# xulinfei1996/koordinator

Measured on AMD Instinct MI355X. Metric: pods scheduled/sec + node-evals/sec (% HBM roofline) at 5k and 100k nodes, higher is better.
Workload: dtype int64; 1 GPU; C2: 10000 pods x 5000 nodes, NodeResourcesFit(LeastAllocated cpu/mem/batch-cpu/batch-mem) + LoadAwareScheduling(defaults) + ElasticQuota(32 leaf quotas); nodes=5000, percentage_of_nodes_to_score=100, parallelism=single-gpu, batch_pods=64, candidates=32

## Files before the change

koordinator_amd/csrc/koordgpu.hip:

```cpp
#include <hip/hip_runtime.h>

#include <algorithm>
#include <chrono>
#include <cmath>
#include <condition_variable>
#include <cstdio>
#include <cstdlib>
#include <cstring>
#include <mutex>
#include <string>
#include <vector>

#include <rccl/rccl.h>

#include "ks_pass.h"
#include "ks_mono.h"
#include "ks_fq.h"
#include "ks_debug.h"
#include "ks_topo.h"
#include "ks_preempt.h"

using namespace ks;

static int64_t env_i64(const char* name, int64_t dflt, int64_t lo, int64_t hi) {
// ... 921 lines not shown
  void* numa_blob = nullptr;
  DevNuma nv{};
  DevNuma* dnv = nullptr;
  char* numa_ckpt = nullptr;
  int64_t numa_policy_nodes = 0;
  bool cpu_bind_labels = false;
  bool cpu_bind_required = false;
  bool val_bind_required = false;
  bool staged_bind_required = false;
  bool cpusets_clobbered = false;
  std::vector<int32_t> h_dev_assumed, h_dev_assumed_ckpt;
  std::vector<int8_t> h_numa_k;
  std::vector<uint16_t> h_dev_ids;
  std::vector<uint8_t> h_pol;
  std::vector<uint8_t> h_dev_held;
  bool dev_held_any = false;
  int64_t* rsv_dald_ckpt = nullptr;
  std::vector<int8_t> h_cpu_nn;
  std::vector<CpuTopo> h_topos;
  std::vector<int8_t> h_topo_dense;
  std::vector<int32_t> h_rsv_node;
  void* dscratch = nullptr;
  size_t dscratch_bytes = 0;
  uint32_t* cpuset_split = nullptr;
  hipStream_t sstream = nullptr;
  hipStream_t cstream = nullptr;
  int32_t* pipe = nullptr;
  unsigned long long* pipe_top = nullptr;
  hipEvent_t pev_sel[kPipeEvents] = {};
  hipEvent_t pev_com[kPipeEvents] = {};
  int64_t pipe_k = 0;
  int32_t pipe_mode = -1;
  bool commit_fq = true;
  void* npod_blob = nullptr;
  DevNodePods npt{};
  int32_t npod_slots = 0;
  PreemptCand* pre_cand = nullptr;
  int32_t* pre_vrank = nullptr;
  uint8_t* pre_status = nullptr;
  PreemptOut* pre_out = nullptr;
  int32_t* pre_victims = nullptr;
  int32_t topo_nkeys = 0, topo_ndom = 1, topo_nprops = 0;
  std::vector<int32_t*> topo_dom_v;
  std::vector<int32_t*> topo_count_v;
  int32_t* topo_dom = nullptr;
  int32_t* topo_count = nullptr;
  long long* topo_zsum = nullptr;
  uint32_t *topo_zpres = nullptr, *topo_zsize = nullptr;
  void* topo_blob = nullptr;
  double* topo_lw = nullptr;
  int32_t topo_nlw = 0;
  TopoScratch* topo_scr = nullptr;
  long long *topo_sraw = nullptr, *topo_iraw = nullptr;
  int32_t topo_k = 1;
  uint32_t* topo_cchunk = nullptr;
  uint2* topo_ct = nullptr;
  int32_t* topo_ccount = nullptr;
  uint64_t *topo_cbound = nullptr, *topo_ctop = nullptr, *topo_csecond = nullptr;
  ks_stats stats{};
  std::vector<hipEvent_t> ev_pool;
};

#define KS_FAIL(ctx, code, ...)                                        \
  do {                                                                 \
    char buf_[512];                                                    \
    snprintf(buf_, sizeof(buf_), __VA_ARGS__);                         \
// ... 185 lines not shown
      g_create_error = "ks_create: TaintToleration / NodeAffinity plugin weight out of range";
      return KS_EINVAL;
    }
  }
  if (cfg->reservation.enable) {
    const int64_t fitla = 100 * ((cfg->fit.enable_score ? cfg->fit.plugin_weight : 0) +
                                 (cfg->loadaware.enable_score ? cfg->loadaware.plugin_weight : 0) +
                                 (cfg->numa.enable ? cfg->numa.plugin_weight : 0) +
                                 (cfg->deviceshare.enable ? cfg->deviceshare.plugin_weight : 0) +
                                 (cfg->balanced.enable ? cfg->balanced.plugin_weight : 0) +
                                 (cfg->taint.enable_score ? cfg->taint.plugin_weight : 0) +
                                 (cfg->affinity.enable_score ? cfg->affinity.plugin_weight : 0));
    if (cfg->reservation.plugin_weight <= fitla || cfg->reservation.plugin_weight > ((int64_t)1 << 40) ||
        (fitla + 1) * (kRsvOrderBase + 1) >= (1 << 26)) {
      g_create_error = "ks_create: Reservation plugin weight must exceed 100 x (Fit + LoadAware weights) (ks_rsv.h ranking)";
      return KS_EUNSUPPORTED;
    }
  }
  int ndev = 0;
  if (hipGetDeviceCount(&ndev) != hipSuccess || ndev == 0) {
    g_create_error = "ks_create: no HIP device available";
    return KS_EHIP;
  }
  if (cfg->device < 0 || cfg->device >= ndev) {
    g_create_error = "ks_create: device ordinal out of range";
    return KS_EINVAL;
  }
  ks_ctx* ctx = new ks_ctx();
  ctx->cfg = *cfg;
  ctx->device = cfg->device;
  ctx->batch = cfg->batch_pods > 0 ? std::min(cfg->batch_pods, kMaxBatch) : 64;
  ctx->k = cfg->candidates > 0 ? std::min(cfg->candidates, kMaxCand) : 32;
  ctx->commit_fq = env_i64("KS_COMMIT_FQ", 1, 0, 1) != 0;
  if (hipSetDevice(ctx->device) != hipSuccess || hipStreamCreateWithFlags(&ctx->stream, hipStreamNonBlocking) != hipSuccess) {
    g_create_error = "ks_create: cannot create HIP stream";
    delete ctx;
    return KS_EHIP;
  }
  void* p = nullptr;
  size_t cand_bytes = (size_t)2 * kMaxBatch * kMaxCand;
  if (dev_alloc(ctx, &p, cand_bytes * 4) != KS_OK) goto fail;
  ctx->cand_chunk = (uint32_t*)p;
  if (dev_alloc(ctx, &p, cand_bytes * 8) != KS_OK) goto fail;
  ctx->cand_t = (uint2*)p;
  if (dev_alloc(ctx, &p, 2 * kMaxBatch * 8) != KS_OK) goto fail;
  ctx->cand_bound = (uint64_t*)p;
  if (dev_alloc(ctx, &p, 2 * kMaxBatch * 8) != KS_OK) goto fail;
  ctx->cand_top = (uint64_t*)p;
  if (dev_alloc(ctx, &p, 2 * kMaxBatch * 8) != KS_OK) goto fail;
  ctx->cand_second = (uint64_t*)p;
  if (dev_alloc(ctx, &p, (size_t)kMaxBatch * kPreRsvM * sizeof(PreRsv)) != KS_OK) goto fail;
  ctx->pre_rsv = (PreRsv*)p;
  if (dev_alloc(ctx, &p, 2 * kMaxBatch * 4) != KS_OK) goto fail;
  ctx->cand_total = (int32_t*)p;
  if (dev_alloc(ctx, &p, 2 * kMaxBatch * 4) != KS_OK) goto fail;
  ctx->cand_count = (int32_t*)p;
  if (dev_alloc(ctx, &p, 64) != KS_OK) goto fail;
  ctx->cursor = (int32_t*)p;
  if (dev_alloc(ctx, &p, 256) != KS_OK) goto fail;
  ctx->counters = (unsigned long long*)p;
  if (dev_alloc(ctx, &p, kNormRows * kMaxBatch * 8) != KS_OK) goto fail;
  ctx->dev_M = (unsigned long long*)p;
  if (hipMemsetAsync(ctx->cand_count, list_fill(), 2 * kMaxBatch * 4, ctx->stream) != hipSuccess ||
      hipMemsetAsync(ctx->cand_chunk, list_fill(), cand_bytes * 4, ctx->stream) != hipSuccess ||
      hipMemsetAsync(ctx->cand_t, list_fill(), cand_bytes * 8, ctx->stream) != hipSuccess ||
      hipStreamSynchronize(ctx->stream) != hipSuccess) {
// ... 2095 lines not shown
  ca.numa_bytes = (int32_t)numa_cache_bytes(ctx);
  ca.nv = ctx->dnv;
  ca.pipe_base = nullptr;
  ca.carry = nullptr;
  ca.pipe_follow = nullptr;
  ca.pipe_after = nullptr;
  ca.top_reset = nullptr;
  ca.pre_rsv = nullptr;
  ca.topo = ctx->cfg.topology.enable && st.topo ? 1 : 0;
  ca.topo_const = (int32_t)(100 * ctx->cfg.topology.spread_weight);
  ca.topo_rec = st.topo;
  ca.topo_props = st.topo_props;
  ca.topo_count = ctx->topo_count;
  ca.topo_npad = ctx->npad;
  ca.topo_best = ctx->topo_scr ? &ctx->topo_scr->best_total : nullptr;
  *smem = commit_layout(ctx->k, ctx->nchunks, *qcache, (size_t)ca.rsv_bytes, (size_t)ca.dev_bytes, (size_t)ca.numa_bytes,
                        ctx->q.q, kernel_feat(ctx) == 0, commit_hint_variant(ctx)).total;
  return ca;
}

static bool mono_commit(const ks_ctx* ctx, bool qcache, size_t* smem) {
  static const int64_t mode = env_i64("KS_COMMIT_GENERAL", 0, 0, 2);
  if (mode == 1 || kernel_feat(ctx) != 0 || !ctx->kc.monotone || ctx->kc.fit_most) return false;
  if (mode == 0 && ctx->kc.quota_enable) return false;
  *smem = mono_layout(ctx->k, ctx->nchunks, qcache, ctx->q.q).total;
  return *smem <= 160 * 1024;
}

static bool fq_commit(const ks_ctx* ctx, bool qcache, bool patch) {
  return ctx->commit_fq && qcache && !patch && kernel_feat(ctx) == 0 && ctx->kc.monotone && !ctx->kc.fit_most &&
         ctx->kc.quota_enable;
}

static FqLaunch fq_launcher(int nsc) { return nsc == 0 ? fq_launch_n0() : (nsc == 2 ? fq_launch_n2() : fq_launch_n4()); }

static bool pre_reserve(const ks_ctx* ctx) {
  static const int64_t env_pre = env_i64("KS_PRE_RSV", 1, 0, 1);
  return env_pre != 0 && ctx->kc.numa_pol;
}

static int commit_attr_set(ks_ctx* ctx) {
  bool qcache = false;
  const int32_t rcap = commit_rcap(ctx, &qcache);
  const size_t smem = commit_layout(ctx->k, ctx->nchunks, qcache, rsv_cache_bytes(ctx, rcap), dev_cache_bytes(ctx),
                                    numa_cache_bytes(ctx), ctx->q.q, kernel_feat(ctx) == 0, commit_hint_variant(ctx)).total;
  if (smem > 160 * 1024)
    KS_FAIL(ctx, KS_EUNSUPPORTED, "too many nodes for the commit kernel's LDS (%lld nodes, %zu B)", (long long)ctx->n, smem);
  hipError_t e = pass_launcher(kernel_feat(ctx), ctx->nsc).commit_attr(qcache, smem);
  if (e != hipSuccess) KS_FAIL(ctx, KS_EHIP, "hipFuncSetAttribute(commit LDS %zu): %s", smem, hipGetErrorString(e));
  if (fq_commit(ctx, qcache, false)) {
    e = fq_launcher(ctx->nsc).commit_attr(smem);
    if (e != hipSuccess) KS_FAIL(ctx, KS_EHIP, "hipFuncSetAttribute(fq commit LDS %zu): %s", smem, hipGetErrorString(e));
  }
  size_t msmem = 0;
  if (mono_commit(ctx, qcache, &msmem)) {
    e = pass_launcher(0, ctx->nsc).commit_mono_attr(qcache, msmem);
    if (e != hipSuccess) KS_FAIL(ctx, KS_EHIP, "hipFuncSetAttribute(mono commit LDS %zu): %s", msmem, hipGetErrorString(e));
  }
  return KS_OK;
}

static int ensure_cpuset_bufs(ks_ctx* ctx, int32_t np) {
  if (!ctx->cfg.numa.enable || ctx->cpuset_cap >= np) return KS_OK;
  void* p = ctx->cpuset_list;
  dev_free(p);
  ctx->cpuset_list = nullptr;
  const int32_t cap = std::max<int32_t>(np, 64);
  const size_t o_n = (size_t)cap * 8, o_out = o_n + 16, o_split = o_out + (size_t)cap * sizeof(CpuSet),
               o_alloc = align16(o_split + (size_t)cap * 4), bytes = o_alloc + (size_t)cap * 2 * kNumaDev * 8;
  if (dev_alloc(ctx, &p, bytes) != KS_OK) return KS_ENOMEM;
  ctx->cpuset_list = (int2*)p;
  ctx->cpuset_n = (int32_t*)((char*)p + o_n);
  ctx->cpuset_out = (CpuSet*)((char*)p + o_out);
  ctx->cpuset_split = (uint32_t*)((char*)p + o_split);
  ctx->numa_alloc = (int64_t*)((char*)p + o_alloc);
  ctx->cpuset_cap = cap;
  return KS_OK;
}

constexpr int kPipeWords = 4 + 1 + kMaxBatch;

static bool pipelined(const ks_ctx* ctx) {
  static const int64_t env_pipe = env_i64("KS_PIPE", 1, 0, 2);
  static const int64_t env_min = env_i64("KS_PIPE_MIN_NODES", 32768, 0, (int64_t)1 << 40);
  const int64_t mode = ctx->pipe_mode >= 0 ? ctx->pipe_mode : env_pipe;
// ... 468 lines not shown
  if (patch)
    if (int rc = fix(); rc != KS_OK) return rc;
  hipStream_t cs = pipe ? ctx->cstream : ctx->stream;
  if (patch) {
  } else if (pipe) {
    HIPCHK(ctx, hipEventRecord(ctx->pev_sel[k % kPipeEvents], ss));
    HIPCHK(ctx, hipStreamWaitEvent(cs, ctx->pev_sel[k % kPipeEvents], 0));
  }
  bool qcache = false;
  size_t smem = 0;
  CommitArgs ca = commit_args(ctx, ctx->st, ctx->np, ctx->batch, &qcache, &smem);
  if (pipe) {
    ca.pipe_base = base;
    ca.carry = carry;
  }
  ca.cand_chunk = cset.chunk;
  ca.cand_t = cset.t;
  ca.cand_bound = cset.bound;
  ca.cand_top = cset.top;
  ca.cand_second = cset.second;
  ca.cand_count = cset.count;
  if (patch) {
    ca.pipe_follow = ctx->pipe + ((k + 1) & 1);
    ca.pipe_after = base;
    ca.cand_top = (const uint64_t*)(ctx->pipe_top + (size_t)(k & 1) * kMaxBatch);
    ca.top_reset = ctx->pipe_top + (size_t)(k & 1) * kMaxBatch;
  }
  size_t msmem = 0;
  const bool mono = mono_commit(ctx, qcache, &msmem);
  if (!mono && !pipe && pl.reserve_pre && pre_reserve(ctx)) ca.pre_rsv = ctx->pre_rsv;
  rec(2, cs);
  if (ca.pre_rsv) HIPCHK(ctx, pl.reserve_pre(ctx->batch, cs, ca));
  if (mono) HIPCHK(ctx, pl.commit_mono(qcache, msmem, cs, ca));
  else if (fq_commit(ctx, qcache, patch)) HIPCHK(ctx, fq_launcher(ctx->nsc).commit(smem, cs, ca));
  else HIPCHK(ctx, pl.commit(qcache, smem, cs, ca));
  rec(2, cs);
  if (pipe) HIPCHK(ctx, hipEventRecord(ctx->pev_com[k % kPipeEvents], cs));
  ctx->pipe_k = k + 1;
  return cores_pass_refresh(ctx);
}

static int schedule_staged_impl(ks_ctx* ctx) {
  if (!ctx->node_blob) KS_FAIL(ctx, KS_ESTATE, "schedule before ks_load_nodes");
  HIPCHK(ctx, hipSetDevice(ctx->device));
  bind_mode(ctx, ctx->staged_bind_required);
  ctx->cpusets_clobbered = false;
  ctx->stats = ks_stats{};
  const int32_t np = ctx->np;
  if (np == 0) return KS_OK;
  {
    if (int rc = commit_attr_set(ctx); rc != KS_OK) return rc;
    hipError_t e = hipSuccess;
    const size_t sel_smem = select_smem(ctx->nchunks);
    if (sel_smem > 160 * 1024) KS_FAIL(ctx, KS_EUNSUPPORTED, "too many nodes for the select kernel's LDS (%lld nodes)", (long long)ctx->n);
    e = hipFuncSetAttribute((const void*)select_kernel, hipFuncAttributeMaxDynamicSharedMemorySize, (int)sel_smem);
    if (e != hipSuccess) KS_FAIL(ctx, KS_EHIP, "hipFuncSetAttribute(select LDS %zu): %s", sel_smem, hipGetErrorString(e));
    if (ctx->kc.dev && !ctx->kc.rsv && !ctx->kc.stat && ctx->dcache_words < (int64_t)kMaxBatch * ctx->npad) {
      void* q = ctx->dcache;
      dev_free(q);
      ctx->dcache = nullptr;
      ctx->dcache_words = 0;
      if (dev_alloc(ctx, &q, (size_t)kMaxBatch * ctx->npad * 8) != KS_OK) return KS_ENOMEM;
      ctx->dcache = (unsigned long long*)q;
      ctx->dcache_words = (int64_t)kMaxBatch * ctx->npad;
    }
    const size_t gb = (size_t)ctx->nranks * ctx->vshards * cand_slot_layout(ctx->k).bytes;
    if (ctx->nranks * ctx->vshards > 1 && ctx->gather_bytes < gb) {
// ... 111 lines not shown
  if (cs != ctx->stream) {
    HIPCHK(ctx, hipEventRecord(ctx->pev_com[0], cs));
    HIPCHK(ctx, hipStreamWaitEvent(ctx->stream, ctx->pev_com[0], 0));
  }
  if (ctx->cpu_loaded && ctx->n > 0) {
    hipLaunchKernelGGL(cpuset_kernel, dim3((unsigned)((ctx->n + 255) / 256)), dim3(256), 0, ctx->stream, ctx->cpu,
                       (const int2*)ctx->cpuset_list, (const int32_t*)ctx->cpuset_n, (const uint32_t*)ctx->cpuset_split,
                       (const PodRec*)ctx->st.recs, ctx->cpuset_out, (const uint32_t*)ctx->d.numa_flags,
                       ctx->d.cpu_cores, (int32_t)(ctx->cfg.numa.numa_scoring_strategy == KS_MOST_ALLOCATED),
                       numa_words(ctx), ctx->nv.npad, ctx->n);
    HIPCHK(ctx, hipGetLastError());
  }
  HIPCHK(ctx, hipEventRecord(t1, ctx->stream));
  unsigned long long cnt[16] = {0};
  HIPCHK(ctx, hipMemcpyAsync(cnt, ctx->counters, sizeof(cnt), hipMemcpyDeviceToHost, ctx->stream));
  HIPCHK(ctx, hipStreamSynchronize(ctx->stream));
  float ms = 0;
  (void)hipEventElapsedTime(&ms, t0, t1);
  ctx->stats.total_ms = ms;
  ctx->stats.passes = (int64_t)cnt[0];
  ctx->stats.cut_passes = (int64_t)cnt[1];
  ctx->stats.rescans = (int64_t)cnt[2];
  ctx->stats.slot_misses = (int64_t)cnt[3];
  ctx->stats.bubble_passes = (int64_t)cnt[4];
  ctx->stats.pre_reserves = (int64_t)cnt[5];
  ctx->stats.pipelined = pipe ? (pipe->patch ? 2 : 1) : 0;
  {
    bool qc = false;
    const int32_t rcap = commit_rcap(ctx, &qc);
    const CommitLayout L = commit_layout(ctx->k, ctx->nchunks, qc, rsv_cache_bytes(ctx, rcap), dev_cache_bytes(ctx),
                                         numa_cache_bytes(ctx), ctx->q.q, kernel_feat(ctx) == 0, commit_hint_variant(ctx));
    ctx->stats.commit_lds_bytes = (int64_t)L.total;
    ctx->stats.commit_helpers = L.hint ? 1 : 0;
  }
  for (int i = 0; i < 8; ++i) ctx->stats.diag[i] = (int64_t)cnt[8 + i];
  for (size_t i = 0; i + 1 < evs.size(); i += 2) {
    float e = 0;
    (void)hipEventElapsedTime(&e, ctx->ev_pool[evs[i].second], ctx->ev_pool[evs[i + 1].second]);
    if (evs[i].first == 0) {
      ctx->stats.sweep_ms += e;
      ctx->stats.sweep_launches += 1;
    } else if (evs[i].first == 1) {
      ctx->stats.select_ms += e;
    } else if (evs[i].first == 3) {
      ctx->stats.fixup_ms += e;
    } else {
      ctx->stats.commit_ms += e;
    }
  }
  int64_t b_node = 8 * 15 + 4 * 3 + (int64_t)ctx->nsc * 16 + (ctx->kc.rsv ? 8 : 0) + (ctx->kc.numa ? 16 : 0) +
                   (ctx->kc.dev ? 4 + (kDevTW + kDevQW) * 8 : 0);
  const int64_t groups = (ctx->batch + ppw - 1) / ppw;
  ctx->stats.sweep_bytes = local_chunks * 64 * b_node * groups + (int64_t)ctx->batch * sizeof(PodRec) + local_chunks * 64 * 4;
  return KS_OK;
}

int ks_schedule_staged(ks_ctx* ctx) {
  if (!ctx) return KS_EINVAL;
  return schedule_staged_impl(ctx);
}

int ks_fetch_results(ks_ctx* ctx, ks_result* out, int32_t p) {
  if (!ctx || !out || p < 0 || p > ctx->np) return ctx ? (ctx->err = "ks_fetch_results: bad args", KS_EINVAL) : KS_EINVAL;
  if (p == 0) return KS_OK;
  HIPCHK(ctx, hipMemcpyAsync(out, ctx->st.results, (size_t)p * sizeof(ks_result), hipMemcpyDeviceToHost, ctx->stream));
  HIPCHK(ctx, hipStreamSynchronize(ctx->stream));
// ... 920 lines not shown
```

koordinator_amd/csrc/ks_fq.h:

```cpp
#pragma once

#include "ks_pass.h"

namespace ks {

struct __attribute__((aligned(16))) FqPod {
  uint32_t qmeta;
  uint32_t flags;
  uint32_t qword;
  int32_t second;
  uint64_t bound, top;
};
static_assert(sizeof(FqPod) == 32, "FqPod layout");
static_assert(kMaxBatch == 64 && kMaxCand <= 64 && kQuotaLdsRows < 0xFFFF && KS_QUOTA_DIMS <= 8, "FqPod packing");

template <int NSC>
__device__ __forceinline__ uint64_t fq_rescan(const DevNodes* dnp, const Cfg& cfg, const PodRec& pod, int64_t chunk,
                                              uint64_t touched_mask, int64_t n) {
  const int lane = threadIdx.x & 63;
  const int64_t node = chunk * 64 + lane;
  asm volatile("" : "+s"(dnp));
  const DevNodes d = *dnp;
  NodeReg<NSC> r;
  load_node<NSC>(cfg, d, node, node < n, r);
  const EvalOut o = eval_pod_node<NSC, false>(cfg, pod, r);
  const bool skip = o.reasons || ((touched_mask >> lane) & 1ull);
  return wave_max_u64(skip ? 0ull : gkey(o.total, node));
}

template <int NSC>
__global__ __launch_bounds__(commit_threads(0)) void commit_fq_kernel(CommitArgs a) {
  constexpr int NT = commit_threads(0);
  extern __shared__ __attribute__((aligned(16))) unsigned char smem_raw[];
  const int32_t K = a.k;
  const CommitLayout lay = commit_layout(K, a.nchunks, true, (size_t)a.rsv_bytes, (size_t)a.dev_bytes, (size_t)a.numa_bytes,
                                         a.q.q, true, false);
  SlotRow* rows = reinterpret_cast<SlotRow*>(smem_raw + lay.rows);
  PodRec* spods = reinterpret_cast<PodRec*>(smem_raw + lay.pods);
  ks_result* sres = reinterpret_cast<ks_result*>(smem_raw + lay.res);
  int64_t* raw = reinterpret_cast<int64_t*>(smem_raw + lay.raw);
  int64_t* rawtop = reinterpret_cast<int64_t*>(smem_raw + lay.rawtop);
  int64_t* rawrun = reinterpret_cast<int64_t*>(smem_raw + lay.rawrun);
  int64_t* pqreq = reinterpret_cast<int64_t*>(smem_raw + lay.pqreq);
  uint2* cand_t = reinterpret_cast<uint2*>(smem_raw + lay.cand_t);
  uint32_t* cand_chunk = reinterpret_cast<uint32_t*>(smem_raw + lay.cand_chunk);
  FqPod* precs = reinterpret_cast<FqPod*>(smem_raw + lay.snuma);
  QuotaRowsLds qview = quota_lds(smem_raw + lay.quota, a.q.q);
  QuotaRowsLds* qlds = &qview;
  unsigned long long* touched = reinterpret_cast<unsigned long long*>(smem_raw + lay.touched);
  int2* hdesc = reinterpret_cast<int2*>(smem_raw + lay.help);
  int32_t* hpend = reinterpret_cast<int32_t*>(smem_raw + lay.help + (size_t)kMaxBatch * 8);
  int32_t* hdone = hpend + 1;
  unsigned long long* hready = reinterpret_cast<unsigned long long*>(smem_raw + lay.help + (size_t)kMaxBatch * 8 + 16);
  const int tid = threadIdx.x;
  const int lane = tid & 63;
  const int32_t cursor0 = __builtin_amdgcn_readfirstlane(*a.cursor);
  if (cursor0 >= a.total_pods) {
    if (threadIdx.x == 0) pipe_next(a, cursor0);
    return;
  }
  if (pipe_bubble(a, cursor0)) return;
  const int32_t np = topo_pass_pods(a, cursor0, min(a.batch, a.total_pods - cursor0));
  if (np == 0) return;
#ifdef KS_COMMIT_STAMPS
  uint64_t ph[8] = {0, 0, 0, 0, 0, 0, 0, 0};
  uint64_t tlast = __builtin_amdgcn_s_memtime();
#define KS_FSTAMP(i)                                   \
  do {                                                 \
    const uint64_t t_ = __builtin_amdgcn_s_memtime(); \
    ph[i] += t_ - tlast;                               \
    tlast = t_;                                        \
  } while (0)
#else
#define KS_FSTAMP(i) \
  do {               \
  } while (0)
#endif

  lds_copy<NT>(cand_chunk, a.cand_chunk, np * K, tid);
  lds_copy<NT>(cand_t, a.cand_t, np * K, tid);
  for (int32_t i = tid; i < np * KS_QUOTA_DIMS; i += NT) {
    const int32_t p = i / KS_QUOTA_DIMS, dd = i - p * KS_QUOTA_DIMS;
    pqreq[i] = a.pq.req[dd][cursor0 + p];
  }
  {
// ... 14 lines not shown
    qlds->limit[i] = a.q.limit[i];
    qlds->used[i] = a.q.used[i];
    qlds->min[i] = a.q.min[i];
    qlds->npused[i] = a.q.npused[i];
  }
  if (tid < 64 && lane < np) {
    const int32_t cnt = a.cand_count[lane];
    const uint64_t second = a.cand_second[lane];
    const uint32_t pmask = a.pq.mask[cursor0 + lane];
    const int32_t quota = a.pods[cursor0 + lane].quota;
    FqPod r;
    r.bound = a.cand_bound[lane];
    r.top = a.cand_top[lane];
    r.flags = a.pods[cursor0 + lane].flags;
    r.qmeta = 0xFFFFu;
    if (quota >= 0) {
      const int32_t pp = a.q.parent[quota];
      r.qmeta = (uint32_t)(pp < 0 ? 0xFFFF : pp) | ((a.q.limit_mask[quota] & 0xFFu) << 16) |
                ((a.q.min_mask[quota] & 0xFFu) << 24);
    }
    r.qword = (uint32_t)(quota < 0 ? 0xFFFF : quota) | ((pmask & 0xFFu) << 16) | ((uint32_t)max(0, min(cnt, 64)) << 24);
    r.second = (int32_t)gkey_node(second);
    precs[lane] = r;
  }
  const void* my_col = nullptr;
  int32_t my_w = 8;
  if (tid < RF_N) {
    my_col = a.rowcols[lane].p;
    my_w = a.rowcols[lane].width;
  }
  if (tid == 0) {
    *hpend = 0;
    *hdone = 0;
    *hready = 0ull;
  }
  __syncthreads();
  if (tid >= 128) return;
  KS_FSTAMP(0);
  Cfg cfg{};
  {
    auto pin = [](int32_t v) {
      asm volatile("" : "+s"(v));
      return v;
    };
    cfg.fit_filter = pin(a.c.fit_filter);
    cfg.fit_score = pin(a.c.fit_score);
    cfg.fw_cpu = pin(a.c.fw_cpu);
    cfg.fw_mem = pin(a.c.fw_mem);
    cfg.fw_eph = pin(a.c.fw_eph);
#pragma unroll
    for (int k = 0; k < NSC; ++k) cfg.fw_sc[k] = pin(a.c.fw_sc[k]);
    cfg.fit_pw = pin(a.c.fit_pw);
    cfg.la_filter = pin(a.c.la_filter);
    cfg.la_score = pin(a.c.la_score);
    cfg.la_prod_usage = pin(a.c.la_prod_usage);
    cfg.lw_cpu = pin(a.c.lw_cpu);
    cfg.lw_mem = pin(a.c.lw_mem);
    cfg.la_pw = pin(a.c.la_pw);
    cfg.quota_enable = 1;
    cfg.quota_parent = pin(a.c.quota_parent);
    cfg.monotone = 1;
  }
  int32_t Kc = K;
  asm volatile("" : "+s"(Kc));

  constexpr int kTerms = ST_NCPU;
  int32_t t_cap = 0, t_req = 0, t_pw = 0, t_pw100 = 0;
  bool t_prod_only = false, t_score = true;
  switch (lane) {
    case ST_CPU: t_cap = RF_ALLOC_CPU; t_req = RF_NZ_CPU; t_pw = 3; t_pw100 = 12; break;
// ... 6 lines not shown
    case ST_LMEM: t_cap = RF_LA_ALLOC_MEM; t_req = RF_TERM_MEM; t_pw = 6; t_pw100 = 16; break;
    case ST_PLCPU: t_cap = RF_LA_ALLOC_CPU; t_req = RF_PTERM_CPU; t_pw = 5; t_pw100 = 15; t_prod_only = true; break;
    case ST_PLMEM: t_cap = RF_LA_ALLOC_MEM; t_req = RF_PTERM_MEM; t_pw = 6; t_pw100 = 16; t_prod_only = true; break;
    case ST_FREE_CPU: t_cap = RF_ALLOC_CPU; t_req = RF_REQ_CPU; t_pw = 0; t_pw100 = 0; t_score = false; break;
    case ST_FREE_MEM: t_cap = RF_ALLOC_MEM; t_req = RF_REQ_MEM; t_pw = 1; t_pw100 = 1; t_score = false; break;
    case ST_FREE_EPH: t_cap = RF_ALLOC_EPH; t_req = RF_REQ_EPH; t_pw = 2; t_pw100 = 2; t_score = false; break;
    case ST_FREE_SC + 0: case ST_FREE_SC + 1: case ST_FREE_SC + 2: case ST_FREE_SC + 3:
      t_cap = RF_ALLOC_SC + (lane - ST_FREE_SC); t_req = RF_REQ_SC + (lane - ST_FREE_SC);
      t_pw = 7 + (lane - ST_FREE_SC); t_pw100 = t_pw; t_score = false; break;
    default: break;
  }
  constexpr int kLaneCounts = ST_N;
  auto build_row = [&](SlotRow* row, const int64_t* src, const int64_t* podw, uint32_t pflags) {
    const bool take = !t_prod_only || (pflags & KS_POD_PROD);
    const int64_t f_cap = src[t_cap], f_req = src[t_req], f_pw = podw[t_pw];
    const int64_t u_bits = src[RF_LA_BITS], u_allowed = src[RF_ALLOWED], u_pods = src[RF_POD_COUNT];
    const int64_t u_acpu = src[RF_ALLOC_CPU], u_amem = src[RF_ALLOC_MEM], u_aeph = src[RF_ALLOC_EPH];
    const int64_t cap = f_cap, req = f_req + (take ? f_pw : 0);
    if (lane < kTerms) {
      Term t;
      t.c = cap;
      t.h = cap - req + ((cap != 0 || !t_score) ? 0 : kNoCap);
      t.hd = cap != 0 ? (double)(cap - req) * 100.0 : 0.0;
      t.r = cap != 0 ? 1.0 / (double)cap : 0.0;
      row->t[lane] = t;
    } else if (lane == kLaneCounts) {
      row->la_bits = (uint32_t)u_bits;
      row->allowed = (int32_t)u_allowed;
      row->pod_count = (int32_t)u_pods + 1;
      row->fit_ws = (u_acpu != 0 ? cfg.fw_cpu : 0) + (u_amem != 0 ? cfg.fw_mem : 0) + (u_aeph != 0 ? cfg.fw_eph : 0);
    }
  };

  if (tid >= 64) {
    int32_t next = 0;
    for (;;) {
      const int32_t pend =
          __builtin_amdgcn_readfirstlane(__hip_atomic_load(hpend, __ATOMIC_ACQUIRE, __HIP_MEMORY_SCOPE_WORKGROUP));
      if (next < pend) {
        const int2 d = hdesc[next];
        const int32_t w = __builtin_amdgcn_readfirstlane(d.y);
        const int32_t s = w & 0xFF, jj = (w >> 8) & 0xFF;
        const int64_t* src = (((w >> 16) & 1) ? rawrun : rawtop) + jj * 32;
        const uint32_t pflags = __builtin_amdgcn_readfirstlane(spods[jj].flags);
        build_row(&rows[s], src, reinterpret_cast<const int64_t*>(&spods[jj]), pflags);
        if (lane == 0)
          __hip_atomic_fetch_or(hready, 1ull << s, __ATOMIC_RELEASE, __HIP_MEMORY_SCOPE_WORKGROUP);
        ++next;
        continue;
      }
      if (__builtin_amdgcn_readfirstlane(__hip_atomic_load(hdone, __ATOMIC_ACQUIRE, __HIP_MEMORY_SCOPE_WORKGROUP)) &&
          next >= __builtin_amdgcn_readfirstlane(__hip_atomic_load(hpend, __ATOMIC_ACQUIRE, __HIP_MEMORY_SCOPE_WORKGROUP)))
        break;
      __builtin_amdgcn_s_sleep(1);
    }
    return;
  }
  int32_t hn = 0;
  uint64_t hown = 0;
  auto wait_rows = [&](uint64_t need) {
    if ((hown & need) == need) return;
    for (;;) {
      const uint64_t r =
          readlane64(__hip_atomic_load(hready, __ATOMIC_ACQUIRE, __HIP_MEMORY_SCOPE_WORKGROUP), 0) | hown;
      if ((r & need) == need) break;
      __builtin_amdgcn_s_sleep(1);
    }
  };

  int32_t snode = -1;
  int32_t nslots = 0;
  int32_t processed = np;
  uint32_t rescans = 0, misses = 0, fast = 0;

  uint32_t st_next = 0, flags_next = 0, qword_next = 0xFFFFu;
  int32_t par_next = -1, second_next = -1;
  uint64_t bound_next = 0;
  int64_t req_next = 0;
  Cands cn{};
  auto lookahead = [&](int32_t j) {
    const uint4 w = *reinterpret_cast<const uint4*>(&precs[j]);
    const ulonglong2 bt = *reinterpret_cast<const ulonglong2*>(&precs[j].bound);
    const uint32_t qm = __builtin_amdgcn_readfirstlane(w.x);
    const uint32_t flags = __builtin_amdgcn_readfirstlane(w.y);
    const uint32_t qw = __builtin_amdgcn_readfirstlane(w.z);
    const bool has_q = (qw & 0xFFFFu) != 0xFFFFu;
    const int32_t qr = has_q ? (int32_t)(qw & 0xFFFFu) : 0;
    const int ld = lane & (KS_QUOTA_DIMS - 1);
    const size_t o = (size_t)qr * KS_QUOTA_DIMS + ld;
    const int64_t req = pqreq[j * KS_QUOTA_DIMS + ld];
    const int64_t u = qlds->used[o], l = qlds->limit[o];
    const int64_t nu = qlds->npused[o], mn = qlds->min[o];
    const uint64_t top = readlane64(bt.y, 0);
    const int32_t tn = top ? (int32_t)gkey_node(top) : 0;
    const uint64_t tw = touched[tn >> 6];
    const uint32_t lm = (qm >> 16) & 0xFFu, mm = qm >> 24;
    const int32_t par = (qm & 0xFFFFu) == 0xFFFFu ? -1 : (int32_t)(qm & 0xFFFFu);
    req_next = req;
    flags_next = flags;
    qword_next = qw;
    par_next = par;
    second_next = w.w;
    bound_next = bt.x;
    st_next = 0;
    cn.fast = false;
    cn.umax = top;
    if (has_q) {
      const uint32_t pmask = (qw >> 16) & 0xFFu;
      const bool in_pod = lane < KS_QUOTA_DIMS && ((pmask >> lane) & 1u);
      if (__ballot(in_pod && ((lm >> lane) & 1u) && (req + u > l))) {
        st_next = KS_S_QUOTA;
      } else if ((flags & KS_POD_NONPREEMPTIBLE) && __ballot(in_pod && ((mm >> lane) & 1u) && (req + nu > mn))) {
        st_next = KS_S_QUOTA_NONPREEMPTIBLE;
      } else if (cfg.quota_parent && par >= 0) {
        st_next = quota_admit(qlds->parent, qlds->limit_mask, qlds->min_mask, qlds->limit, qlds->used, qlds->min,
                              qlds->npused, true, qr, 0u, pmask, req, true);
      }
    }
    KS_FSTAMP(6);
    if (st_next) return;
    if (top && !((tw >> (tn & 63)) & 1ull)) {
      cn.fast = true;
      return;
    }
    cn = resolve_cands(cand_chunk, cand_t, touched, j, Kc, (int32_t)(qw >> 24));
  };
  lookahead(0);
  KS_FSTAMP(1);

  for (int32_t j = 0; j < np; ++j) {
    const uint32_t st = st_next;
    const Cands cj = cn;
    const int32_t qpar = par_next;
    const int64_t qreq_j = req_next;
    const uint32_t pflags = flags_next, qword = qword_next;
    if (st) {
      if (lane == 0) sres[j] = ks_result{-1, st, 0, -1, 0, 0, 0};
      goto next_pod;
    }
    {
      uint64_t best;
      int32_t node;
      if (cj.fast) {
        best = cj.umax;
        ++fast;
        KS_FSTAMP(2);
        node = (int32_t)gkey_node(best);
        const int32_t s = nslots++;
        if (lane == s) snode = node;
        if (lane == 0) {
          atomicOr(&touched[node >> 6], 1ull << (node & 63));
          hdesc[hn] = make_int2(node, s | (j << 8));
          __hip_atomic_store(hpend, hn + 1, __ATOMIC_RELEASE, __HIP_MEMORY_SCOPE_WORKGROUP);
        }
        ++hn;
      } else {
        PodRec pod = spods[j];
        pod.flags = pflags;
        uint64_t key_mod = 0;
        wait_rows(nslots >= 64 ? ~0ull : ((1ull << nslots) - 1));
        if (lane < nslots) {
          NodeReg<NSC> r;
          slot_to_reg<NSC>(rows[lane], r);
          const EvalOut o = eval_pod_node<NSC, false>(cfg, pod, r);
          if (o.reasons == 0) key_mod = gkey(o.total, snode);
        }
        best = umax64(cj.umax, wave_max_u64(key_mod));
        KS_FSTAMP(2);
        uint64_t need = __ballot(!cj.exact && cj.valid && cj.ub > best);
        while (need) {
          const uint64_t kmax = wave_max_u64(((need >> lane) & 1ull) ? cj.ub : 0ull);
          const int sel = __ffsll((long long)__ballot(((need >> lane) & 1ull) && cj.ub == kmax)) - 1;
          const int64_t c = (int64_t)(uint32_t)__shfl((int)cj.chunk, sel, 64);
          const uint64_t v = fq_rescan<NSC>(a.dn, cfg, pod, c, touched[c], a.n);
          ++rescans;
          best = umax64(best, v);
          need &= ~(1ull << sel);
          need &= __ballot(cj.ub > best);
        }
        if (best < readlane64(bound_next, 0)) {
          processed = j;
          break;
        }
        KS_FSTAMP(3);
        if (best == 0) {
          if (lane == 0) sres[j] = ks_result{-1, KS_S_UNSCHEDULABLE, 0, -1, 0, 0, 0};
          goto next_pod;
        }
        node = (int32_t)gkey_node(best);
        const int64_t* podw = reinterpret_cast<const int64_t*>(&spods[j]);
        int32_t s = __ffsll((long long)__ballot(snode == node)) - 1;
        if (s < 0) {
          s = nslots++;
          if (lane == s) snode = node;
          if (lane == 0) atomicOr(&touched[node >> 6], 1ull << (node & 63));
          if (node == __builtin_amdgcn_readfirstlane(second_next)) {
            if (lane == 0) {
              hdesc[hn] = make_int2(node, s | (j << 8) | (1 << 16));
              __hip_atomic_store(hpend, hn + 1, __ATOMIC_RELEASE, __HIP_MEMORY_SCOPE_WORKGROUP);
            }
            ++hn;
          } else {
            ++misses;
            if (lane < RF_N) raw[lane] = load_field(my_col, my_w, node);
            hown |= 1ull << s;
            build_row(&rows[s], raw, podw, pflags);
          }
        } else {
          wait_rows(1ull << s);
          SlotRow* row = &rows[s];
          const bool take = !t_prod_only || (pflags & KS_POD_PROD);
          if (lane < kTerms) {
            if (take) term_take(row->t[lane], podw[t_pw], __longlong_as_double(podw[t_pw100]));
          } else if (lane == kLaneCounts) {
            row->pod_count += 1;
          }
        }
      }
      KS_FSTAMP(4);
      if (lane == 0) sres[j] = ks_result{node, KS_S_SCHEDULED, gkey_score(best), -1, 0, 0, 0};
      if ((qword & 0xFFFFu) != 0xFFFFu) {
        const int32_t qrow = (int32_t)(qword & 0xFFFFu);
        const uint32_t pmask = (qword >> 16) & 0xFFu;
        if (lane < KS_QUOTA_DIMS && ((pmask >> lane) & 1u)) {
          const bool np_ = (pflags & KS_POD_NONPREEMPTIBLE) != 0;
          atomicAdd((unsigned long long*)&qlds->used[(size_t)qrow * KS_QUOTA_DIMS + lane], (unsigned long long)qreq_j);
          if (np_) atomicAdd((unsigned long long*)&qlds->npused[(size_t)qrow * KS_QUOTA_DIMS + lane], (unsigned long long)qreq_j);
          for (int32_t cur = qpar; cur >= 0;) {
            const int32_t up = qlds->parent[cur];
            atomicAdd((unsigned long long*)&qlds->used[(size_t)cur * KS_QUOTA_DIMS + lane], (unsigned long long)qreq_j);
            if (np_) atomicAdd((unsigned long long*)&qlds->npused[(size_t)cur * KS_QUOTA_DIMS + lane], (unsigned long long)qreq_j);
            cur = up;
          }
        }
      }
      KS_FSTAMP(5);
    }
  next_pod:
    if (j + 1 < np) lookahead(j + 1);
    KS_FSTAMP(1);
  }
  KS_FSTAMP(6);
  if (lane == 0) __hip_atomic_store(hdone, 1, __ATOMIC_RELEASE, __HIP_MEMORY_SCOPE_WORKGROUP);
  wait_rows(nslots >= 64 ? ~0ull : ((1ull << nslots) - 1));
  if (lane < processed) {
    ks_result r = sres[lane];
    topo_writeback(a, cursor0 + lane, r);
    a.results[cursor0 + lane] = r;
  }
// ... 6 lines not shown
    gst(d.req_eph + node, r.t[ST_FREE_EPH].c - r.t[ST_FREE_EPH].h);
    gst(d.nz_cpu + node, term_requested(r.t[ST_CPU]));
    gst(d.nz_mem + node, term_requested(r.t[ST_MEM]));
#pragma unroll
    for (int k = 0; k < KS_MAX_SCALARS; ++k) gst(d.req_sc[k] + node, r.t[ST_FREE_SC + k].c - r.t[ST_FREE_SC + k].h);
    gst(d.pod_count + node, r.pod_count);
    gst(d.la_term_cpu + node, term_requested(r.t[ST_LCPU]));
    gst(d.la_term_mem + node, term_requested(r.t[ST_LMEM]));
    gst(d.la_pterm_cpu + node, term_requested(r.t[ST_PLCPU]));
    gst(d.la_pterm_mem + node, term_requested(r.t[ST_PLMEM]));
  }
  for (int32_t i = lane; i < a.q.q * KS_QUOTA_DIMS; i += 64) {
    a.q.used[i] = qlds->used[i];
    a.q.npused[i] = qlds->npused[i];
  }
  pipe_carry(a, nslots, snode);
  if (a.top_reset) a.top_reset[lane] = 0ull;
  if (lane == 0) {
    *a.cursor = cursor0 + processed;
    pipe_next(a, cursor0 + processed);
    atomicAdd(&a.counters[0], 1ull);
    if (processed < np) atomicAdd(&a.counters[1], 1ull);
    atomicAdd(&a.counters[2], (unsigned long long)rescans);
    atomicAdd(&a.counters[3], (unsigned long long)misses);
    atomicAdd(&a.counters[15], (unsigned long long)fast);
#ifdef KS_COMMIT_STAMPS
    for (int i = 0; i < 7; ++i) atomicAdd(&a.counters[8 + i], (unsigned long long)ph[i]);
#endif
  }
#undef KS_FSTAMP
}

struct FqLaunch {
  hipError_t (*commit)(size_t smem, hipStream_t s, const CommitArgs& a);
  hipError_t (*commit_attr)(size_t smem);
};
FqLaunch fq_launch_n0();
FqLaunch fq_launch_n2();
FqLaunch fq_launch_n4();

}
```

koordinator_amd/csrc/ks_pass.h:

```cpp
#pragma once

#include <hip/hip_runtime.h>

#include <type_traits>

#include "ks_device.h"
#include "ks_rsv.h"
#include "ks_dev.h"
#include "ks_cpuset.h"
#include "ks_numa.h"
#include "ks_topo.h"

namespace ks {

__device__ __forceinline__ uint64_t local_gkey(uint32_t loc, int64_t chunk) {
  if (loc == 0) return 0;
  const int64_t node = chunk * 64 + (63 - (int64_t)(loc & 63u));
  return ((uint64_t)(loc >> 6) << 32) | (uint64_t)(0xFFFFFFFFu - (uint32_t)node);
}


struct SweepArgs {
  const DevNodes* __restrict__ dn;
  const DevRsv* __restrict__ rv;
// ... 325 lines not shown

__host__ __device__ inline size_t quota_lds_bytes(int32_t q) {
  const size_t r = (size_t)(q > 0 ? q : 1);
  return (r * 12 + 15) / 16 * 16 + r * KS_QUOTA_DIMS * 32;
}

__device__ __forceinline__ QuotaRowsLds quota_lds(unsigned char* p, int32_t q) {
  const size_t r = (size_t)(q > 0 ? q : 1);
  QuotaRowsLds v;
  v.parent = reinterpret_cast<int32_t*>(p);
  v.limit_mask = reinterpret_cast<uint32_t*>(p + r * 4);
  v.min_mask = reinterpret_cast<uint32_t*>(p + r * 8);
  int64_t* w = reinterpret_cast<int64_t*>(p + (r * 12 + 15) / 16 * 16);
  v.limit = w;
  v.used = w + r * KS_QUOTA_DIMS;
  v.min = w + 2 * r * KS_QUOTA_DIMS;
  v.npused = w + 3 * r * KS_QUOTA_DIMS;
  return v;
}

constexpr size_t kHelpBytes = (size_t)kMaxBatch * 8 + 16 + 16;
struct DevVar {
  uint32_t sel;
  uint32_t reasons;
  int32_t raw;
  uint32_t _pad;
};
constexpr int kDevVars = 4;
constexpr size_t kHelpHintBytes = (size_t)kMaxBatch * (24 + kDevVars * 16) + 64;
static_assert(sizeof(DevHints) == 24 && sizeof(DevVar) == 16, "help region");

struct CommitLayout {
  size_t rows, pods, res, raw, rawtop, rawrun, pqreq, cand_t, cand_chunk, scls, snuma, srcnt, srec, sdev, snp, quota, help,
      touched, total;
  bool hint;
};

__host__ __device__ inline size_t align16(size_t x) { return (x + 15) / 16 * 16; }

__host__ __device__ inline CommitLayout commit_layout(int32_t k, int64_t nchunks, bool qc, size_t rsv_bytes = 0,
                                                      size_t dev_bytes = 0, size_t numa_bytes = 0,
                                                      int32_t qrows = kQuotaLdsRows, bool run = false,
                                                      bool hint_ok = false) {
  CommitLayout L;
  size_t o = 0;
  L.rows = o;
  o += (size_t)kMaxBatch * sizeof(SlotRow);
  L.pods = o;
  o += (size_t)kMaxBatch * sizeof(PodRec);
  L.res = o;
  o += align16((size_t)kMaxBatch * sizeof(ks_result));
  L.raw = o;
  o += 32 * 8;
  L.rawtop = o;
  o += (size_t)kMaxBatch * 32 * 8;
  L.rawrun = o;
  if (run) o += (size_t)kMaxBatch * 32 * 8;
  L.pqreq = o;
  o += (size_t)kMaxBatch * KS_QUOTA_DIMS * 8;
  L.cand_t = o;
  o += (size_t)kMaxBatch * k * sizeof(uint2);
  L.cand_chunk = o;
  o += align16((size_t)kMaxBatch * k * 4);
  L.scls = o;
  o += (size_t)kMaxBatch * 8;
  L.snuma = o;
  o += (size_t)kMaxBatch * 32;
  L.srcnt = o;
  o += (size_t)kMaxBatch * 8;
  L.srec = o;
  o += align16(rsv_bytes);
  L.sdev = o;
  o += align16(dev_bytes);
  L.snp = o;
  o += align16(numa_bytes);
  L.quota = o;
  if (qc) o += align16(quota_lds_bytes(qrows));
  L.help = o;
  L.hint = hint_ok && dev_bytes && numa_bytes && o + kHelpHintBytes + (size_t)nchunks * 8 <= (size_t)160 * 1024;
  o += L.hint ? kHelpHintBytes : kHelpBytes;
  L.touched = o;
  o += (size_t)nchunks * 8;
  L.total = o;
  return L;
}

template <typename P32, typename PU32, typename P64>
__device__ __forceinline__ uint32_t quota_admit(P32 parent, PU32 limit_mask, PU32 min_mask, P64 limit, P64 used,
                                                P64 minv, P64 npused, bool check_parent, int32_t quota,
                                                uint32_t flags, uint32_t pmask, int64_t req,
                                                bool skip_leaf = false) {
  const int lane = threadIdx.x & 63;
  const bool in_pod = lane < KS_QUOTA_DIMS && ((pmask >> lane) & 1u);
  const int ld = lane < KS_QUOTA_DIMS ? lane : 0;
  const size_t o = (size_t)quota * KS_QUOTA_DIMS + ld;
  if (!skip_leaf) {
    const uint32_t lm = limit_mask[quota];
    const int64_t u = used[o], l = limit[o];
    const bool bad = in_pod && ((lm >> lane) & 1u) && (req + u > l);
    if (__ballot(bad)) return KS_S_QUOTA;
  }
  if (flags & KS_POD_NONPREEMPTIBLE) {
    const uint32_t mm = min_mask[quota];
    const int64_t u = npused[o], m = minv[o];
    const bool bad = in_pod && ((mm >> lane) & 1u) && (req + u > m);
    if (__ballot(bad)) return KS_S_QUOTA_NONPREEMPTIBLE;
  }
  if (check_parent) {
    for (int32_t cur = parent[quota]; cur >= 0; cur = parent[cur]) {
      const size_t oc = (size_t)cur * KS_QUOTA_DIMS + ld;
      const bool bad = in_pod && ((limit_mask[cur] >> lane) & 1u) && (req + used[oc] > limit[oc]);
      if (__ballot(bad)) return KS_S_QUOTA | KS_S_QUOTA_PARENT;
    }
  }
  return 0;
// ... 1467 lines not shown
```

koordinator_amd/csrc/ks_variant.hip:

```cpp
#include "ks_pass.h"
#include "ks_mono.h"
#include "ks_fq.h"

#if !defined(KS_FEAT) || !defined(KS_NSC)
#error "compile with -DKS_FEAT=<feature bits> -DKS_NSC=<0|2|4>"
#endif

#define KS_CAT2(a, b) a##b
#define KS_CAT(a, b) KS_CAT2(a, b)

namespace ks {
namespace {

constexpr int F = KS_FEAT;

constexpr int NSC = KS_NSC;

hipError_t sweep(int blocks, hipStream_t s, const SweepArgs& a) {
  hipLaunchKernelGGL((sweep_kernel<NSC, F>), dim3(blocks), dim3(256), 0, s, a);
  return hipGetLastError();
}

hipError_t commit(bool qc, size_t smem, hipStream_t s, const CommitArgs& a) {
  if (qc) hipLaunchKernelGGL((commit_kernel<NSC, true, F>), dim3(1), dim3(commit_threads(F)), smem, s, a);
  else hipLaunchKernelGGL((commit_kernel<NSC, false, F>), dim3(1), dim3(commit_threads(F)), smem, s, a);
  return hipGetLastError();
}

hipError_t commit_attr(bool qc, size_t smem) {
  const void* fn = qc ? (const void*)commit_kernel<NSC, true, F> : (const void*)commit_kernel<NSC, false, F>;
  return hipFuncSetAttribute(fn, hipFuncAttributeMaxDynamicSharedMemorySize, (int)smem);
}

#if KS_FEAT == 0
hipError_t commit_mono(bool qc, size_t smem, hipStream_t s, const CommitArgs& a) {
  if (qc) hipLaunchKernelGGL((commit_mono_kernel<NSC, true>), dim3(1), dim3(commit_threads(0)), smem, s, a);
  else hipLaunchKernelGGL((commit_mono_kernel<NSC, false>), dim3(1), dim3(commit_threads(0)), smem, s, a);
  return hipGetLastError();
}

hipError_t commit_mono_attr(bool qc, size_t smem) {
  const void* fn = qc ? (const void*)commit_mono_kernel<NSC, true> : (const void*)commit_mono_kernel<NSC, false>;
  return hipFuncSetAttribute(fn, hipFuncAttributeMaxDynamicSharedMemorySize, (int)smem);
}

hipError_t commit_fq(size_t smem, hipStream_t s, const CommitArgs& a) {
  hipLaunchKernelGGL((commit_fq_kernel<NSC>), dim3(1), dim3(commit_threads(0)), smem, s, a);
  return hipGetLastError();
}

hipError_t commit_fq_attr(size_t smem) {
  return hipFuncSetAttribute((const void*)commit_fq_kernel<NSC>, hipFuncAttributeMaxDynamicSharedMemorySize, (int)smem);
}
#endif

#if (KS_FEAT & 8) != 0
hipError_t reserve_pre(int blocks, hipStream_t s, const CommitArgs& a) {
  hipLaunchKernelGGL((reserve_pre_kernel<F>), dim3(blocks), dim3(64), 0, s, a);
  return hipGetLastError();
}
#endif

}

PassLaunch KS_CAT(KS_CAT(KS_CAT(pass_launch_f, KS_FEAT), _n), KS_NSC)() {
#if KS_FEAT == 0
  return PassLaunch{sweep, commit, commit_attr, commit_mono, commit_mono_attr, nullptr};
#elif (KS_FEAT & 8) != 0
  return PassLaunch{sweep, commit, commit_attr, nullptr, nullptr, reserve_pre};
#else
  return PassLaunch{sweep, commit, commit_attr, nullptr, nullptr, nullptr};
#endif
}

#if KS_FEAT == 0
FqLaunch KS_CAT(fq_launch_n, KS_NSC)() { return FqLaunch{commit_fq, commit_fq_attr}; }
#endif

}
```

Before: 546,800 pods/s.

## Precompute slot-pod eval keys in a helper wave of the fq commit kernel

Adds a KEYS variant of the fused-quota commit kernel. A third helper wave evaluates every later batch pod against each newly built or updated slot row and stores the keys in an LDS table. The main wave then reads these precomputed keys instead of waiting for rows and running eval_pod_node for all slots on the critical path. The cost is an extra LDS table of about 16KB, an extra active wave, and more spin-wait synchronisation between waves, which could add latency if the helper falls behind.

```diff
diff --git a/koordinator_amd/csrc/koordgpu.hip b/koordinator_amd/csrc/koordgpu.hip
--- a/koordinator_amd/csrc/koordgpu.hip
+++ b/koordinator_amd/csrc/koordgpu.hip
@@ -977,6 +977,7 @@
   int64_t pipe_k = 0;
   int32_t pipe_mode = -1;
   bool commit_fq = true;
+  bool fq_keys = true;
   void* npod_blob = nullptr;
   DevNodePods npt{};
   int32_t npod_slots = 0;
@@ -1228,6 +1229,7 @@
   ctx->batch = cfg->batch_pods > 0 ? std::min(cfg->batch_pods, kMaxBatch) : 64;
   ctx->k = cfg->candidates > 0 ? std::min(cfg->candidates, kMaxCand) : 32;
   ctx->commit_fq = env_i64("KS_COMMIT_FQ", 1, 0, 1) != 0;
+  ctx->fq_keys = env_i64("KS_FQ_KEYS", 1, 0, 1) != 0;
   if (hipSetDevice(ctx->device) != hipSuccess || hipStreamCreateWithFlags(&ctx->stream, hipStreamNonBlocking) != hipSuccess) {
     g_create_error = "ks_create: cannot create HIP stream";
     delete ctx;
@@ -3389,6 +3391,15 @@
          ctx->kc.quota_enable;
 }
 
+static bool fq_keys(const ks_ctx* ctx, bool qcache, bool patch, size_t* smem) {
+  if (!ctx->fq_keys || !fq_commit(ctx, qcache, patch)) return false;
+  const size_t t = commit_layout(ctx->k, ctx->nchunks, true, 0, dev_cache_bytes(ctx), numa_cache_bytes(ctx), ctx->q.q, true,
+                                 false, true).total;
+  if (t > 160 * 1024) return false;
+  *smem = t;
+  return true;
+}
+
 static FqLaunch fq_launcher(int nsc) { return nsc == 0 ? fq_launch_n0() : (nsc == 2 ? fq_launch_n2() : fq_launch_n4()); }
 
 static bool pre_reserve(const ks_ctx* ctx) {
@@ -3406,8 +3417,10 @@
   hipError_t e = pass_launcher(kernel_feat(ctx), ctx->nsc).commit_attr(qcache, smem);
   if (e != hipSuccess) KS_FAIL(ctx, KS_EHIP, "hipFuncSetAttribute(commit LDS %zu): %s", smem, hipGetErrorString(e));
   if (fq_commit(ctx, qcache, false)) {
-    e = fq_launcher(ctx->nsc).commit_attr(smem);
-    if (e != hipSuccess) KS_FAIL(ctx, KS_EHIP, "hipFuncSetAttribute(fq commit LDS %zu): %s", smem, hipGetErrorString(e));
+    size_t fsmem = smem;
+    const bool keys = fq_keys(ctx, qcache, false, &fsmem);
+    e = fq_launcher(ctx->nsc).commit_attr(keys, fsmem);
+    if (e != hipSuccess) KS_FAIL(ctx, KS_EHIP, "hipFuncSetAttribute(fq commit LDS %zu): %s", fsmem, hipGetErrorString(e));
   }
   size_t msmem = 0;
   if (mono_commit(ctx, qcache, &msmem)) {
@@ -3942,7 +3955,11 @@
   rec(2, cs);
   if (ca.pre_rsv) HIPCHK(ctx, pl.reserve_pre(ctx->batch, cs, ca));
   if (mono) HIPCHK(ctx, pl.commit_mono(qcache, msmem, cs, ca));
-  else if (fq_commit(ctx, qcache, patch)) HIPCHK(ctx, fq_launcher(ctx->nsc).commit(smem, cs, ca));
+  else if (fq_commit(ctx, qcache, patch)) {
+    size_t fsmem = smem;
+    const bool keys = fq_keys(ctx, qcache, patch, &fsmem);
+    HIPCHK(ctx, fq_launcher(ctx->nsc).commit(keys, fsmem, cs, ca));
+  }
   else HIPCHK(ctx, pl.commit(qcache, smem, cs, ca));
   rec(2, cs);
   if (pipe) HIPCHK(ctx, hipEventRecord(ctx->pev_com[k % kPipeEvents], cs));
@@ -4120,6 +4137,11 @@
                                          numa_cache_bytes(ctx), ctx->q.q, kernel_feat(ctx) == 0, commit_hint_variant(ctx));
     ctx->stats.commit_lds_bytes = (int64_t)L.total;
     ctx->stats.commit_helpers = L.hint ? 1 : 0;
+    size_t fsmem = 0, msmem = 0;
+    if (!mono_commit(ctx, qc, &msmem) && fq_keys(ctx, qc, pipe && pipe->patch, &fsmem)) {
+      ctx->stats.commit_lds_bytes = (int64_t)fsmem;
+      ctx->stats.commit_helpers = 2;
+    }
   }
   for (int i = 0; i < 8; ++i) ctx->stats.diag[i] = (int64_t)cnt[8 + i];
   for (size_t i = 0; i + 1 < evs.size(); i += 2) {
diff --git a/koordinator_amd/csrc/ks_fq.h b/koordinator_amd/csrc/ks_fq.h
--- a/koordinator_amd/csrc/ks_fq.h
+++ b/koordinator_amd/csrc/ks_fq.h
@@ -28,13 +28,13 @@
   return wave_max_u64(skip ? 0ull : gkey(o.total, node));
 }
 
-template <int NSC>
+template <int NSC, bool KEYS>
 __global__ __launch_bounds__(commit_threads(0)) void commit_fq_kernel(CommitArgs a) {
   constexpr int NT = commit_threads(0);
   extern __shared__ __attribute__((aligned(16))) unsigned char smem_raw[];
   const int32_t K = a.k;
   const CommitLayout lay = commit_layout(K, a.nchunks, true, (size_t)a.rsv_bytes, (size_t)a.dev_bytes, (size_t)a.numa_bytes,
-                                         a.q.q, true, false);
+                                         a.q.q, true, false, KEYS);
   SlotRow* rows = reinterpret_cast<SlotRow*>(smem_raw + lay.rows);
   PodRec* spods = reinterpret_cast<PodRec*>(smem_raw + lay.pods);
   ks_result* sres = reinterpret_cast<ks_result*>(smem_raw + lay.res);
@@ -51,6 +51,8 @@
   int2* hdesc = reinterpret_cast<int2*>(smem_raw + lay.help);
   int32_t* hpend = reinterpret_cast<int32_t*>(smem_raw + lay.help + (size_t)kMaxBatch * 8);
   int32_t* hdone = hpend + 1;
+  int32_t* heval = hpend + 2;
+  uint32_t* skey = reinterpret_cast<uint32_t*>(smem_raw + lay.skey);
   unsigned long long* hready = reinterpret_cast<unsigned long long*>(smem_raw + lay.help + (size_t)kMaxBatch * 8 + 16);
   const int tid = threadIdx.x;
   const int lane = tid & 63;
@@ -131,10 +133,11 @@
   if (tid == 0) {
     *hpend = 0;
     *hdone = 0;
+    *heval = 0;
     *hready = 0ull;
   }
   __syncthreads();
-  if (tid >= 128) return;
+  if (tid >= (KEYS ? 192 : 128)) return;
   KS_FSTAMP(0);
   Cfg cfg{};
   {
@@ -207,6 +210,34 @@
     }
   };
 
+  if (KEYS && tid >= 128) {
+    const int32_t pl = min(lane, np - 1);
+    const PodRec pod = spods[pl];
+    int32_t next = 0;
+    for (;;) {
+      if (__builtin_amdgcn_readfirstlane(__hip_atomic_load(hdone, __ATOMIC_ACQUIRE, __HIP_MEMORY_SCOPE_WORKGROUP))) break;
+      const int32_t pend =
+          __builtin_amdgcn_readfirstlane(__hip_atomic_load(hpend, __ATOMIC_ACQUIRE, __HIP_MEMORY_SCOPE_WORKGROUP));
+      if (next >= pend) {
+        __builtin_amdgcn_s_sleep(1);
+        continue;
+      }
+      const int32_t w = __builtin_amdgcn_readfirstlane(hdesc[next].y);
+      const int32_t s = w & 0xFF, jj = (w >> 8) & 0xFF;
+      if (!((w >> 17) & 1) &&
+          !((readlane64(__hip_atomic_load(hready, __ATOMIC_ACQUIRE, __HIP_MEMORY_SCOPE_WORKGROUP), 0) >> s) & 1ull)) {
+        __builtin_amdgcn_s_sleep(1);
+        continue;
+      }
+      NodeReg<NSC> r;
+      slot_to_reg<NSC>(rows[s], r);
+      const EvalOut o = eval_pod_node<NSC, false>(cfg, pod, r);
+      if (lane > jj && lane < np) skey[s * kSlotKeyStride + lane] = o.reasons == 0 ? (uint32_t)(o.total + 1) : 0u;
+      ++next;
+      if (lane == 0) __hip_atomic_store(heval, next, __ATOMIC_RELEASE, __HIP_MEMORY_SCOPE_WORKGROUP);
+    }
+    return;
+  }
   if (tid >= 64) {
     int32_t next = 0;
     for (;;) {
@@ -215,6 +246,10 @@
       if (next < pend) {
         const int2 d = hdesc[next];
         const int32_t w = __builtin_amdgcn_readfirstlane(d.y);
+        if (KEYS && ((w >> 17) & 1)) {
+          ++next;
+          continue;
+        }
         const int32_t s = w & 0xFF, jj = (w >> 8) & 0xFF;
         const int64_t* src = (((w >> 16) & 1) ? rawrun : rawtop) + jj * 32;
         const uint32_t pflags = __builtin_amdgcn_readfirstlane(spods[jj].flags);
@@ -241,6 +276,17 @@
       if ((r & need) == need) break;
       __builtin_amdgcn_s_sleep(1);
     }
+  };
+  auto wait_keys = [&]() {
+    while (__builtin_amdgcn_readfirstlane(__hip_atomic_load(heval, __ATOMIC_ACQUIRE, __HIP_MEMORY_SCOPE_WORKGROUP)) < hn)
+      __builtin_amdgcn_s_sleep(1);
+  };
+  auto issue_built = [&](int32_t node, int32_t s, int32_t j) {
+    if (lane == 0) {
+      hdesc[hn] = make_int2(node, s | (j << 8) | (1 << 17));
+      __hip_atomic_store(hpend, hn + 1, __ATOMIC_RELEASE, __HIP_MEMORY_SCOPE_WORKGROUP);
+    }
+    ++hn;
   };
 
   int32_t snode = -1;
@@ -292,7 +338,6 @@
                               qlds->npused, true, qr, 0u, pmask, req, true);
       }
     }
-    KS_FSTAMP(6);
     if (st_next) return;
     if (top && !((tw >> (tn & 63)) & 1ull)) {
       cn.fast = true;
@@ -330,20 +375,32 @@
         }
         ++hn;
       } else {
-        PodRec pod = spods[j];
-        pod.flags = pflags;
         uint64_t key_mod = 0;
-        wait_rows(nslots >= 64 ? ~0ull : ((1ull << nslots) - 1));
-        if (lane < nslots) {
-          NodeReg<NSC> r;
-          slot_to_reg<NSC>(rows[lane], r);
-          const EvalOut o = eval_pod_node<NSC, false>(cfg, pod, r);
-          if (o.reasons == 0) key_mod = gkey(o.total, snode);
+        if (KEYS) {
+          wait_keys();
+          KS_FSTAMP(6);
+          if (lane < nslots) {
+            const uint32_t v = skey[lane * kSlotKeyStride + j];
+            if (v) key_mod = ((uint64_t)v << 32) | (uint64_t)(0xFFFFFFFFu - (uint32_t)snode);
+          }
+        } else {
+          wait_rows(nslots >= 64 ? ~0ull : ((1ull << nslots) - 1));
+          KS_FSTAMP(6);
+          if (lane < nslots) {
+            PodRec pod = spods[j];
+            pod.flags = pflags;
+            NodeReg<NSC> r;
+            slot_to_reg<NSC>(rows[lane], r);
+            const EvalOut o = eval_pod_node<NSC, false>(cfg, pod, r);
+            if (o.reasons == 0) key_mod = gkey(o.total, snode);
+          }
         }
         best = umax64(cj.umax, wave_max_u64(key_mod));
         KS_FSTAMP(2);
         uint64_t need = __ballot(!cj.exact && cj.valid && cj.ub > best);
         while (need) {
+          PodRec pod = spods[j];
+          pod.flags = pflags;
           const uint64_t kmax = wave_max_u64(((need >> lane) & 1ull) ? cj.ub : 0ull);
           const int sel = __ffsll((long long)__ballot(((need >> lane) & 1ull) && cj.ub == kmax)) - 1;
           const int64_t c = (int64_t)(uint32_t)__shfl((int)cj.chunk, sel, 64);
@@ -380,6 +437,7 @@
             if (lane < RF_N) raw[lane] = load_field(my_col, my_w, node);
             hown |= 1ull << s;
             build_row(&rows[s], raw, podw, pflags);
+            if (KEYS) issue_built(node, s, j);
           }
         } else {
           wait_rows(1ull << s);
@@ -390,6 +448,7 @@
           } else if (lane == kLaneCounts) {
             row->pod_count += 1;
           }
+          if (KEYS) issue_built(node, s, j);
         }
       }
       KS_FSTAMP(4);
@@ -462,8 +521,8 @@
 }
 
 struct FqLaunch {
-  hipError_t (*commit)(size_t smem, hipStream_t s, const CommitArgs& a);
-  hipError_t (*commit_attr)(size_t smem);
+  hipError_t (*commit)(bool keys, size_t smem, hipStream_t s, const CommitArgs& a);
+  hipError_t (*commit_attr)(bool keys, size_t smem);
 };
 FqLaunch fq_launch_n0();
 FqLaunch fq_launch_n2();
diff --git a/koordinator_amd/csrc/ks_pass.h b/koordinator_amd/csrc/ks_pass.h
--- a/koordinator_amd/csrc/ks_pass.h
+++ b/koordinator_amd/csrc/ks_pass.h
@@ -381,16 +381,19 @@
 
 struct CommitLayout {
   size_t rows, pods, res, raw, rawtop, rawrun, pqreq, cand_t, cand_chunk, scls, snuma, srcnt, srec, sdev, snp, quota, help,
-      touched, total;
+      touched, skey, total;
   bool hint;
 };
 
 __host__ __device__ inline size_t align16(size_t x) { return (x + 15) / 16 * 16; }
+
+constexpr int kSlotKeyStride = kMaxBatch + 1;
+constexpr size_t kSlotKeyBytes = (size_t)kMaxBatch * kSlotKeyStride * 4;
 
 __host__ __device__ inline CommitLayout commit_layout(int32_t k, int64_t nchunks, bool qc, size_t rsv_bytes = 0,
                                                       size_t dev_bytes = 0, size_t numa_bytes = 0,
                                                       int32_t qrows = kQuotaLdsRows, bool run = false,
-                                                      bool hint_ok = false) {
+                                                      bool hint_ok = false, bool slot_keys = false) {
   CommitLayout L;
   size_t o = 0;
   L.rows = o;
@@ -430,6 +433,8 @@
   o += L.hint ? kHelpHintBytes : kHelpBytes;
   L.touched = o;
   o += (size_t)nchunks * 8;
+  L.skey = o;
+  if (slot_keys) o += kSlotKeyBytes;
   L.total = o;
   return L;
 }
diff --git a/koordinator_amd/csrc/ks_variant.hip b/koordinator_amd/csrc/ks_variant.hip
--- a/koordinator_amd/csrc/ks_variant.hip
+++ b/koordinator_amd/csrc/ks_variant.hip
@@ -44,13 +44,15 @@
   return hipFuncSetAttribute(fn, hipFuncAttributeMaxDynamicSharedMemorySize, (int)smem);
 }
 
-hipError_t commit_fq(size_t smem, hipStream_t s, const CommitArgs& a) {
-  hipLaunchKernelGGL((commit_fq_kernel<NSC>), dim3(1), dim3(commit_threads(0)), smem, s, a);
+hipError_t commit_fq(bool keys, size_t smem, hipStream_t s, const CommitArgs& a) {
+  if (keys) hipLaunchKernelGGL((commit_fq_kernel<NSC, true>), dim3(1), dim3(commit_threads(0)), smem, s, a);
+  else hipLaunchKernelGGL((commit_fq_kernel<NSC, false>), dim3(1), dim3(commit_threads(0)), smem, s, a);
   return hipGetLastError();
 }
 
-hipError_t commit_fq_attr(size_t smem) {
-  return hipFuncSetAttribute((const void*)commit_fq_kernel<NSC>, hipFuncAttributeMaxDynamicSharedMemorySize, (int)smem);
+hipError_t commit_fq_attr(bool keys, size_t smem) {
+  const void* fn = keys ? (const void*)commit_fq_kernel<NSC, true> : (const void*)commit_fq_kernel<NSC, false>;
+  return hipFuncSetAttribute(fn, hipFuncAttributeMaxDynamicSharedMemorySize, (int)smem);
 }
 #endif
 
```

Measured after the change: 573,800 pods/s, median of 6. 1.05x the previous value.
